# HongjianFang/DSurfTomo

Hardware: AMD Instinct MI355X
Metric: source-period FMM solves/sec on NxN grid; travel-time max-abs-err vs ref (higher is better)
Workload: dtype f32

## Files before the change

### dsurftomo_amd/csrc/bundle_kernel.hip

```cpp
#include "kernels.h"
#include "receiver_core.h"
#include "wave_ops.h"

namespace dsa {

namespace {

__device__ __forceinline__ unsigned bf2u(float f) { return __float_as_uint(f); }
__device__ __forceinline__ float bu2f(unsigned u) { return __uint_as_float(u); }

enum { BC_READY = 0, BC_READY_ODD, BC_TMIN, BC_THETA, BC_FREEZE, BC_HASH, BC_OVERFLOW, BC_CUR, BC_STALE, BC_STALEMIN, BC_SLOWN, BC_FARALL, BC_COUNT };
constexpr int kFarStrikes = 8;
constexpr int kBundleCycleRounds = 8;
constexpr float kStaleWindows = 16.0f;
constexpr int kStaleRounds = 6;

typedef __attribute__((address_space(1))) unsigned long long BGU64;
typedef __attribute__((address_space(1))) char BGChar;
typedef __attribute__((address_space(1))) float BGF32;
typedef __attribute__((address_space(1))) const float BGCF32;
typedef float __attribute__((ext_vector_type(4))) BV4;
typedef __attribute__((address_space(1))) BV4 BGV4;
typedef float __attribute__((ext_vector_type(2))) BV2;
template <int MPL> struct BMem;
// ... 18 lines not shown

template <int CH>
__device__ __forceinline__ unsigned node_or(unsigned v)
{
    if (CH >= 2) v |= (unsigned)__builtin_amdgcn_update_dpp(0, (int)v, 0xb1, 0xf, 0xf, false);
    if (CH >= 4) v |= (unsigned)__builtin_amdgcn_update_dpp(0, (int)v, 0x4e, 0xf, 0xf, false);
    if (CH >= 8) v |= (unsigned)__builtin_amdgcn_update_dpp(0, (int)v, 0x141, 0xf, 0xf, false);
    return v;
}

}

#ifdef DSA_BUNDLE_WAVES
#define DSA_BUNDLE_OCC(G, NT, MPL) __attribute__((amdgpu_waves_per_eu(DSA_BUNDLE_WAVES, DSA_BUNDLE_WAVES)))
#else
#define DSA_BUNDLE_OCC(G, NT, MPL) __attribute__((amdgpu_waves_per_eu((((NT) == 256 && ((MPL) == 2 || (G) == 16)) || (NT) == 768) ? 3 : 1, (((NT) == 256 && ((MPL) == 2 || (G) == 16)) || (NT) == 768) ? 3 : 2)))
#endif
template <int G, int NT, int MPL = 4, bool TIE = false>
__global__ __launch_bounds__(NT) DSA_BUNDLE_OCC(G, NT, MPL) void k_fim_bundle(const FimBundle* __restrict__ bundles, const FimProblem* __restrict__ problems,
                                                    const FimEnds* __restrict__ ends)
{
    constexpr int NW = NT / 64;
    constexpr int CH = G / MPL;
    typedef typename BMem<MPL>::V BV;
    typedef typename BMem<MPL>::GV BGV;
    constexpr int NPW = 64 / CH;
    constexpr unsigned GB = G * 4u * DSA_BSTRIDE;
    extern __shared__ unsigned dyn_lds[];
    __shared__ int sc[BC_COUNT];
    constexpr int kWaveBuf = 256, kTileBuf = NT > 256 ? 128 : 256, kClrWords = 4;
    __shared__ int wbuf[NW * kWaveBuf];
// ... 904 lines not shown
            if (TIE && pm->tie) { pm->tie[4] = freezes; pm->tie[7] = cand_g ? __hip_atomic_load(cand_g, __ATOMIC_RELAXED, __HIP_MEMORY_SCOPE_AGENT) : -1; }
            if (failed && pm->info[2] != -2) pm->info[2] = -1;
            if (sc[BC_OVERFLOW]) pm->info[2] = -2;
        }
        if (E->rays) {
            const GridDesc g = E->g;
            for (int r = tid; r < E->nrays; r += NT) {
                const RayDesc rd = E->rays[r];
                if (!(rd.flags & kRayTime)) continue;
                float t;
                if (!receiver_time(g, E->scx, E->scz, rd, (const float*)Bslot + m, E->veln, E->dpl, &t, G * DSA_BSTRIDE)) atomicExch(E->err, E->ray0 + r + 1);
                E->out[rd.data] = t;
            }
        }
    }
    {
        __shared__ float* s_dst[kBundleMax];
        __syncthreads();
        if (tid < kBundleMax) s_dst[tid] = tid < nmem ? problems[s_member[tid]].Tc : nullptr;
        __syncthreads();
        bool any_dst = false;
        for (int m = 0; m < nmem; ++m) any_dst = any_dst || s_dst[m] != nullptr;
        if (any_dst)
            for (int i = tid; i < ntile * kTileRecs; i += NT) {
#pragma unroll
                for (int c4 = 0; c4 < G / 4; ++c4) {
                    const BV4 v = *(BGV4*)(Bb + (unsigned)i * GB + (unsigned)c4 * 16u);
                    BGF32* d;
                    if ((d = (BGF32*)s_dst[4 * c4 + 0])) d[i] = fabsf(v.x);
                    if ((d = (BGF32*)s_dst[4 * c4 + 1])) d[i] = fabsf(v.y);
                    if ((d = (BGF32*)s_dst[4 * c4 + 2])) d[i] = fabsf(v.z);
                    if ((d = (BGF32*)s_dst[4 * c4 + 3])) d[i] = fabsf(v.w);
// ... 4 lines not shown
        __threadfence();
        __syncthreads();
        if (tid == 0) __hip_atomic_store(&bd->slot_busy[my_slot], 0, __ATOMIC_RELEASE, __HIP_MEMORY_SCOPE_AGENT);
    }
}

size_t bundle_lds_bytes(int tile_words) { return (size_t)tile_words * 4; }

void launch_fim_bundles(const FimBundle* d_bundles, int nbundles, int G, int threads, const FimProblem* d_problems, const FimEnds* d_ends, int tile_words, hipStream_t stream, int members_per_lane, bool tie)
{
    if (nbundles <= 0) return;
    const size_t lds = bundle_lds_bytes(tile_words);
#define DSA_LAUNCH_BUNDLE_T(GG, TT, MM, TIE_) hipLaunchKernelGGL((k_fim_bundle<GG, TT, MM, TIE_>), dim3(nbundles), dim3(TT), lds, stream, d_bundles, d_problems, d_ends)
#define DSA_LAUNCH_BUNDLE_G(TT, MM, TIE_) { if (G == 16) DSA_LAUNCH_BUNDLE_T(16, TT, MM, TIE_); else if (G == 8) DSA_LAUNCH_BUNDLE_T(8, TT, MM, TIE_); else DSA_LAUNCH_BUNDLE_T(4, TT, MM, TIE_); }
#define DSA_LAUNCH_BUNDLE(TT, MM) { if (tie) DSA_LAUNCH_BUNDLE_G(TT, MM, true) else DSA_LAUNCH_BUNDLE_G(TT, MM, false) }
    if (members_per_lane == 2 && threads == 256) DSA_LAUNCH_BUNDLE(256, 2)
    else if (threads == 512) DSA_LAUNCH_BUNDLE(512, 4)
    else if (threads == 768) DSA_LAUNCH_BUNDLE(768, 4)
    else DSA_LAUNCH_BUNDLE(256, 4)
#undef DSA_LAUNCH_BUNDLE_T
#undef DSA_LAUNCH_BUNDLE_G
#undef DSA_LAUNCH_BUNDLE
}

__global__ void k_interleave_maps(const float* __restrict__ slow_all, size_t field_stride, int np, float* __restrict__ slowI)
{
    const size_t i = (size_t)blockIdx.x * blockDim.x + threadIdx.x;
    if (i >= field_stride * (size_t)np) return;
    const size_t id = i / (size_t)np;
    const int m = (int)(i - id * (size_t)np);
    slowI[i] = slow_all[(size_t)m * field_stride + id];
}

template <int G>
__global__ void k_bundle_refined_slowness(const FimBundle* __restrict__ bundles, const FimProblem* __restrict__ problems, int nrec, float* __restrict__ slowI)
{
    const FimBundle* const bd = bundles + blockIdx.y;
    const int i = blockIdx.x * blockDim.x + threadIdx.x;
    if (i >= nrec * G) return;
    const int id = i / G, m = i - id * G;
    const int mm = m < bd->nmem ? m : 0;
    slowI[((size_t)blockIdx.y * nrec + id) * G + m] = problems[bd->member[mm]].slow[id];
}
template <int G>
__global__ void k_bundle_export_records(const FimBundle* __restrict__ bundles, const FimProblem* __restrict__ problems, int nrec)
{
    const FimBundle* const bd = bundles + blockIdx.y;
    const int i = blockIdx.x * blockDim.x + threadIdx.x;
    if (i >= nrec * G) return;
    const int id = i / G, m = i - id * G;
    if (m >= bd->nmem) return;
    const FimProblem* const pm = problems + bd->member[m];
    if (pm->ended && *pm->ended) return;
    const float v = bd->B[(size_t)bd->slot * bd->b_stride + (size_t)id * G * DSA_BSTRIDE + m];
    Rec r{ v, v };
    if (__builtin_signbit(v)) {
        bool pinned = false;
        const float tau = exc_find(bd->exc + (size_t)bd->slot * bd->exc_stride, bd->exc_log2cap, id * G + m, &pinned);
        r.T = pinned ? v : -v; r.tau = tau;
    }
    pm->F[id] = r;
}

void launch_bundle_refined_slowness(const FimBundle* d_bundles, int nbundles, int G, const FimProblem* d_problems, int nrec, float* d_slowI, hipStream_t stream)
{
    if (nbundles <= 0) return;
    const dim3 grid((unsigned)((nrec * G + 255) / 256), (unsigned)nbundles), block(256);
    if (G == 16) hipLaunchKernelGGL(k_bundle_refined_slowness<16>, grid, block, 0, stream, d_bundles, d_problems, nrec, d_slowI);
    else if (G == 8) hipLaunchKernelGGL(k_bundle_refined_slowness<8>, grid, block, 0, stream, d_bundles, d_problems, nrec, d_slowI);
    else hipLaunchKernelGGL(k_bundle_refined_slowness<4>, grid, block, 0, stream, d_bundles, d_problems, nrec, d_slowI);
}

void launch_bundle_export_records(const FimBundle* d_bundles, int nbundles, int G, const FimProblem* d_problems, int nrec, hipStream_t stream)
{
    if (nbundles <= 0) return;
    const dim3 grid((unsigned)((nrec * G + 255) / 256), (unsigned)nbundles), block(256);
    if (G == 16) hipLaunchKernelGGL(k_bundle_export_records<16>, grid, block, 0, stream, d_bundles, d_problems, nrec);
    else if (G == 8) hipLaunchKernelGGL(k_bundle_export_records<8>, grid, block, 0, stream, d_bundles, d_problems, nrec);
    else hipLaunchKernelGGL(k_bundle_export_records<4>, grid, block, 0, stream, d_bundles, d_problems, nrec);
}

void launch_interleave_maps(const float* d_slow_all, size_t field_stride, int np, float* d_slowI, hipStream_t stream)
{
    const size_t n = field_stride * (size_t)np;
    if (n == 0) return;
    hipLaunchKernelGGL(k_interleave_maps, dim3((unsigned)((n + 255) / 256)), dim3(256), 0, stream, d_slow_all, field_stride, np, d_slowI);
}

}
```

### dsurftomo_amd/csrc/engine.h

```cpp
#pragma once

#include <hip/hip_runtime.h>

#include <string>
#include <vector>

#include "bundle_plan.h"
#include "host_geometry.h"
#include "kernels.h"

namespace dsa {

template <class T>
struct DevBuf {
    T* p = nullptr;
    size_t cap = 0;
    void release() { if (p) (void)hipFree(p); p = nullptr; cap = 0; }
};

template <class T>
struct OwnedBuf : DevBuf<T> {
    OwnedBuf() = default;
    OwnedBuf(const OwnedBuf&) = delete;
    OwnedBuf& operator=(const OwnedBuf&) = delete;
// ... 73 lines not shown
    float bundle_window_opt = 0.0f;
    int bundle_G_now = 0;
    int bundle_threads_opt = 0;
    int bundle_max_rounds = 0;
    int bundle_mpl = 0;
    bool bundle_wide = false;
    int bundle_mpl_now = 4, bundle_mpl_b = 2;
    int bundle_threads_b = 256;
    int bundle_tail_opt = 1;
    int bundle_far_all = 0;
    int bundles_a = 0, bundles_b = 0, bundle_Gb = 0;
    hipStream_t stream2 = nullptr;
    hipEvent_t ev_b0 = nullptr, ev_b1 = nullptr;
    hipError_t make_stream2();
    int bundle_refined_opt = 1;
    bool refined_bundles_failed = false;
    bool refined_bundles_now = false;
    std::vector<FimBundle> h_bundles_r;
    OwnedBuf<FimBundle> bundles_r_d;
    OwnedBuf<FimEnds> ends_r;
    OwnedBuf<float> Br_pool, slowIr;
    OwnedBuf<unsigned long long> exc_br;
    OwnedBuf<int> lists_br, cand_br;
    size_t slowIr_off_b = 0;
    int bundle_pool_opt = 0;
    OwnedBuf<float> slowI, B_pool;
    bool slowI_ready = false;
    bool bundles_failed = false;
    OwnedBuf<unsigned long long> exc_b;
    OwnedBuf<int> lists_b, bpool_gen, member_flag, cand_b;
// ... 261 lines not shown
```

### dsurftomo_amd/csrc/engine.hip

```cpp
#include <hip/hip_runtime.h>

#include <algorithm>
#include <chrono>
#include <cmath>
#include <cstdarg>
#include <cstdio>
#include <cstring>
#include <string>
#include <map>
#include <vector>

#include "../../include/dsurftomo_amd.h"
#include "engine.h"
#include "spmv_state.h"
#include "column_system.h"
#include "column_radial.h"
#include "column_lateral.h"
#include "column_radial_lateral.h"
#include "column_sample.h"

namespace dsa {

static std::string g_create_error;

// ... 1311 lines not shown
           b(rst) + b(cst) + b(cinit) + b(heap) + b(flags) + b(T_c) + b(exc_c) + b(W_c) + b(seed_c) + b(nseed_c) + b(launch_rank) + b(prob_r) + b(prob_c) +
           b(info) + b(clocks) + b(tieinfo) + b(xinfo) + b(x_units) + b(B_pool) + b(exc_b) + b(lists_b) + b(bpool_gen) + b(bundles_d) + b(member_flag);
}

float Engine::bundle_window() const
{
    if (bundle_window_opt > 0.0f) return bundle_window_opt;
    if (bundle_wide && bundle_G_now > 0) return bundle_G_now < 16 ? 1.75f : 1.0f;
    return 0.6f;
}

float Engine::bundle_window_tail() const
{
    if (bundle_window_opt > 0.0f) return bundle_window_opt;
    return bundle_threads_b == 768 && bundle_threads() == 256 ? 1.0f : bundle_window();
}

int Engine::bundle_threads() const
{
    if (bundle_threads_opt == 256 || bundle_threads_opt == 512 || bundle_threads_opt == 768) return bundle_threads_opt;
    if (std::max(g.nnx, g.nnz) > 1500) return 768;
    return bundle_wide ? 768 : 256;
}

BundleOptions Engine::bundle_options() const
{
    return { bundle_opt, bundle_mpl, bundle_tail_opt, bundle_order_opt, bundle_threads(), bundle_threads_opt == 0 };
}

BatchPtrs Engine::batch() const
// ... 135 lines not shown
        if (plan_bundles(first, n, bundle_off_chunk ? 0 : bundle_G, &nsolo, &nbundles) != 0) return status;
        const bool refined_b = nbundles > 0 && refined_bundles_now && !bundle_off_chunk;
        const double bundle_mb = nbundles ? (double)(B_pool.cap * 4 + exc_b.cap * 8 + lists_b.cap * 4 + slowI.cap * 4 + cand_b.cap * 4 + Br_pool.cap * 4 + exc_br.cap * 8 + lists_br.cap * 4 + cand_br.cap * 4 + slowIr.cap * 4) / 1.0e6 : 0.0;
        launch_make_problems(g, b, n, slow.p, nrec_c, risti_c.p, window_r, window_c, prob_r.p, prob_c.p, info.p, clocks.p, launch_rank.p,
                             detect ? tieinfo.p : nullptr, tie_threshold, ends_c.p, fused_times ? rays.p : nullptr, veln.p, nfield, dpl, out.p, err.p,
                             nbundles ? member_flag.p : nullptr, bundle_window() * cell_c, bundle_max_rounds, stream, bundle_window_tail() * cell_c,
                             refined_b ? ends_r.p : nullptr);
        FimLaunch sr = shape_r, sc = shape_c;
        sr.tie = sc.tie = detect ? 1 : 0;
        launch_refine(g, b, n, velv.p, (size_t)g.nx * g.ny, rbasis.p, stream);
        if (exact_ties != 2) launch_refined_startup(g, b, n, stream);
        HIP_TRY(this, hipEventRecord(events[2], stream));
        if (exact_ties != 2 && refined_b) {
            launch_fim(prob_r.p, nsolo, sr, stream);
            const int cnt[2] = { bundles_a, nbundles - bundles_a }, GG[2] = { bundle_G, bundle_Gb }, mpl[2] = { bundle_mpl_now, bundles_b > 0 && bundle_threads_b == 256 ? bundle_mpl_b : bundle_mpl_of(bundle_options(), bundle_Gb ? bundle_Gb : bundle_G, nbundles) };
            for (int q = 0; q < 2; ++q) {
                if (cnt[q] <= 0) continue;
                const FimBundle* const bq = bundles_r_d.p + (q ? bundles_a : 0);
                launch_bundle_refined_slowness(bq, cnt[q], GG[q], prob_r.p, kRefRecs, slowIr.p + (q ? slowIr_off_b : 0), stream);
                launch_fim_bundles(bq, cnt[q], GG[q], 256, prob_r.p, ends_r.p, sr.tile_words, stream, GG[q] == 16 ? 4 : mpl[q], detect);
                launch_bundle_export_records(bq, cnt[q], GG[q], prob_r.p, kRefRecs, stream);
            }
        } else if (exact_ties != 2) launch_fim(prob_r.p, n, sr, stream);
        HIP_TRY(this, hipEventRecord(events[3], stream));
        if (exact_ties != 2) {
            const bool replay = detect && handoff_replay;
            if (replay) HIP_TRY(this, hipMemsetAsync(replay_list.p, 0, sizeof(int32_t), stream));
            launch_handoff(g, b, n, stream, detect ? tieinfo.p : nullptr, tie_threshold, replay ? replay_list.p : nullptr, kHandoffReplayCap, replay_scratch.p, xinfo.p);
            launch_coarse_march(g, b, n, slow.p, nrec_c, risti_c.p, stream, detect ? tieinfo.p : nullptr);
        }
        HIP_TRY(this, hipEventRecord(events[4], stream));
        if (exact_ties != 2) {
            launch_fim(prob_c.p, nsolo, sc, stream, ends_c.p);
            if (nbundles && bundles_b > 0) {
                if (!stream2) HIP_TRY(this, make_stream2());
                HIP_TRY(this, hipEventRecord(ev_b0, stream));
                launch_fim_bundles(bundles_d.p, bundles_a, bundle_G, bundle_threads(), prob_c.p, ends_c.p, sc.tile_words, stream, bundle_mpl_now, detect);
                HIP_TRY(this, hipStreamWaitEvent(stream2, ev_b0, 0));
                launch_fim_bundles(bundles_d.p + bundles_a, bundles_b, bundle_Gb, bundle_threads_b, prob_c.p, ends_c.p, sc.tile_words, stream2, bundle_mpl_b, detect);
                HIP_TRY(this, hipEventRecord(ev_b1, stream2));
                HIP_TRY(this, hipStreamWaitEvent(stream, ev_b1, 0));
            } else if (nbundles) launch_fim_bundles(bundles_d.p, nbundles, bundle_G, bundle_threads(), prob_c.p, ends_c.p, sc.tile_words, stream, bundle_mpl_now, detect);
        }
        HIP_TRY(this, hipEventRecord(events[5], stream));
        if (exact_ties) {
            std::vector<int> xl;
            if (exact_ties == 2) { xl.resize((size_t)n); for (int u = 0; u < n; ++u) xl[(size_t)u] = u; }
            else {
                std::vector<int32_t> h_tie((size_t)n * kTieWords), h_inf((size_t)n * 16);
                HIP_TRY(this, hipMemcpyAsync(h_tie.data(), tieinfo.p, (size_t)n * kTieWords * 4, hipMemcpyDeviceToHost, stream));
                HIP_TRY(this, hipMemcpyAsync(h_inf.data(), info.p, (size_t)n * 64, hipMemcpyDeviceToHost, stream));
                int32_t h_replayed = 0;
                if (handoff_replay) HIP_TRY(this, hipMemcpyAsync(&h_replayed, replay_list.p, 4, hipMemcpyDeviceToHost, stream));
                HIP_TRY(this, hipStreamSynchronize(stream));
                stats[DSA_STAT_HANDOFFS_REPLAYED] += (double)std::min<int32_t>(h_replayed, kHandoffReplayCap);
                bool will_redo = false;
                for (int u = 0; u < n && !will_redo; ++u) {
                    const int32_t* fi = &h_inf[(size_t)u * 16];
                    const bool member = nbundles > 0 && h_member_flag[(size_t)u] != 0;
                    will_redo = fi[10] == -2 || (refined_b && member && fi[2] < 0) || (member && fi[10] == -1);
                }
                if (!will_redo) {
                    const std::vector<char> fl = tie_verdicts(first, n, h_tie.data(), h_inf.data(), nbundles > 0);
                    for (int u = 0; u < n; ++u) if (fl[(size_t)u]) { h_unit_flags[(size_t)(first + u)] |= 1; xl.push_back(u); }
                }
                stats[DSA_STAT_TIE_UNITS] += (double)xl.size();
            }
            if (!xl.empty()) {
                const auto w0 = std::chrono::steady_clock::now();
                const bool times_only = !rows && !keep_fields;
                bool compact = exact_ties == 1 ? n <= pool_slots : (!exact_fused || n <= pool_slots);
                if (times_only && exact_tiles_opt == 1) compact = false;
                marched_in_tiles = false;
                if (run_exact(first, n, xl, exact_fused || exact_ties == 1, compact, times_only) != 0) return status;
                stats[DSA_STAT_MS_EXACT] += std::chrono::duration<double, std::milli>(std::chrono::steady_clock::now() - w0).count();
            }
        }
        const int r0 = h_src[first].first_ray;
        const int r1 = h_src[first + n - 1].first_ray + h_src[first + n - 1].nrec;
        if (!fused_times && !exact_fused && r1 > r0) launch_srtimes_chunk(r0, r1 - r0, first);
        HIP_TRY(this, hipEventRecord(events[6], stream));
        HIP_TRY(this, hipGetLastError());
        h_info.resize((size_t)n * 16);
        h_flags.resize((size_t)n * 4);
        std::vector<int32_t> h_tie0;
        if (exact_ties == 0 && detect) { h_tie0.resize((size_t)n * kTieWords); HIP_TRY(this, hipMemcpyAsync(h_tie0.data(), tieinfo.p, (size_t)n * kTieWords * 4, hipMemcpyDeviceToHost, stream)); }
        HIP_TRY(this, hipMemcpyAsync(h_info.data(), info.p, (size_t)n * 16 * 4, hipMemcpyDeviceToHost, stream));
        HIP_TRY(this, hipMemcpyAsync(h_flags.data(), flags.p, (size_t)n * 4 * 4, hipMemcpyDeviceToHost, stream));
        if (dsurf && r1 > r0) {
            const int d0 = h_rays[r0].data, d1 = h_rays[r1 - 1].data + 1;
            HIP_TRY(this, hipMemcpyAsync(dsurf + d0, out.p + d0, (size_t)(d1 - d0) * 4, hipMemcpyDeviceToHost, stream));
        }
        std::vector<unsigned long long> h_clk((size_t)n * kClockSlots);
        HIP_TRY(this, hipMemcpyAsync(h_clk.data(), clocks.p, (size_t)n * kClockSlots * 8, hipMemcpyDeviceToHost, stream));
        HIP_TRY(this, hipStreamSynchronize(stream));
        for (int u = 0; u < n; ++u) {
            for (int q = 0; q < 6; ++q) phase_ticks[q] += (double)h_clk[(size_t)u * kClockSlots + q];
            phase_ticks[7] += (double)h_clk[(size_t)u * kClockSlots + 7];
            phase_ticks[6] = std::max(phase_ticks[6], (double)h_clk[(size_t)u * kClockSlots + 6]);
            for (int q = 8; q < kClockSlots; ++q) phase_ticks[q] += (double)h_clk[(size_t)u * kClockSlots + q];
        }
        float ms = 0;
        float a = 0, c2 = 0, d = 0;
        HIP_TRY(this, hipEventElapsedTime(&ms, events[2], events[3])); stats[DSA_STAT_MS_FIM_REFINED] += ms;
        HIP_TRY(this, hipEventElapsedTime(&ms, events[4], events[5])); stats[DSA_STAT_MS_FIM_COARSE] += ms;
        HIP_TRY(this, hipEventElapsedTime(&a, events[1], events[2]));
        HIP_TRY(this, hipEventElapsedTime(&c2, events[3], events[4]));
        HIP_TRY(this, hipEventElapsedTime(&d, events[5], events[6]));
        stats[DSA_STAT_MS_STAGES] += a + c2 + d;
        stats[DSA_STAT_LAUNCHES_FIM_COARSE] += 1;
        for (int u = 0; u < n; ++u) {
            const int32_t* fi = &h_info[(size_t)u * 16];
            if (fi[10] != -2) continue;
            const size_t grown_bytes = (size_t)pool_slots * (((size_t)8 << (exc_log2cap + 2)) - ((size_t)8 << exc_log2cap));
            size_t free_b = 0, total_b = 0;
            HIP_TRY(this, hipMemGetInfo(&free_b, &total_b));
            if (exc_log2cap + 2 > 26 || grown_bytes + ((size_t)pool_slots << exc_log2cap) * 8 > free_b || ensure(exc_c, (size_t)pool_slots << (exc_log2cap + 2))) {
                fail(DSA_ERR_INTERNAL, "unit %d: the exception table of the compact field overflowed (%d entries) and cannot grow", first + u, 1 << exc_log2cap);
                return DSA_ERR_INTERNAL;
            }
            exc_log2cap += 2;
            exc_log2cap_grown = exc_log2cap;
            per_slot_bytes += grown_bytes / (size_t)pool_slots;
            stats[DSA_STAT_RESCANS] += 1;
// ... 662 lines not shown
    if (n == "fim_lds_pad" && value >= 0 && value <= 64 * 1024) { en->planned = false; en->fim_lds_pad = (int)value; return 0; }
    if (n == "fim_sorted" && (value == 0 || value == 1)) { en->planned = false; en->fim_sorted = (int)value; return 0; }
    if (n == "ray_path_cap" && value >= 0 && value <= (1 << 24)) { en->ray_path_cap = (int)value; return 0; }
    if (n == "disp_group_shift" && value >= -1 && value <= 3) { en->disp_group_shift = (int)value; return 0; }
    if (n == "disp_layers_lds" && (value == -1 || value == 0 || value == 1)) { en->disp_layers_lds = (int)value; return 0; }
    if (n == "exc_log2cap" && (value == 0 || (value >= 6 && value <= 24))) { en->planned = false; en->exc_log2cap_opt = (int)value; return 0; }
    if (n == "rows_on_device" && (value == 0 || value == 1)) { en->rows_on_device = value != 0; return 0; }
    if (n == "lsmr_device_vectors" && (value == 0 || value == 1)) { en->lsmr_device_vectors = (int)value; return 0; }
    if (n == "field_pool" && value >= -1) { en->planned = false; en->field_pool_opt = (int)value; return 0; }
    if (n == "ray_lanes" && (value == 0 || value == 1 || value == 4)) { en->ray_lanes_opt = (int)value; return 0; }
    if (n == "bundle_window_cells" && value >= 0) { en->bundle_window_opt = (float)value; return 0; }
    if (n == "bundle_threads" && (value == 0 || value == 256 || value == 512 || value == 768)) { en->bundle_threads_opt = (int)value; return 0; }
    if (n == "bundle_max_rounds" && value >= 0) { en->bundle_max_rounds = (int)value; return 0; }
    if (n == "bundle_tail" && (value == 0 || value == 1)) { en->bundle_tail_opt = (int)value; return 0; }
    if (n == "bundle_refined" && (value == 0 || value == 1 || value == 2)) { en->bundle_refined_opt = (int)value; return 0; }
    if (n == "bundle_far_all" && (value == 0 || value == 1)) { en->bundle_far_all = (int)value; return 0; }
    if (n == "bundle_pool" && value >= 0) { en->bundle_pool_opt = (int)value; return 0; }
    if (n == "bundle_members_per_lane" && (value == 0 || value == 4 || value == 2)) { en->bundle_mpl = (int)value; return 0; }
    if (n == "bundle" && (value == 0 || value == 1 || value == 4 || value == 8 || value == 16)) { en->planned = false; en->bundle_opt = (int)value; return 0; }
    if (n == "exact_ties" && (value == 0 || value == 1 || value == 2)) { en->exact_ties = (int)value; return 0; }
    if (n == "tie_threshold" && value >= 0) { en->tie_threshold = (float)value; return 0; }
    if (n == "tie_detect" && (value == 0 || value == 1)) { en->tie_detect = (int)value; return 0; }
    if (n == "tie_sum_threshold" && value >= 0) { en->tie_sum_threshold = (float)value; return 0; }
    if (n == "tie_count_threshold" && value >= 0) { en->tie_count_threshold = (int)value; return 0; }
    if (n == "tie_frozen_bundles" && (value == 0 || value == 1)) { en->tie_frozen_bundles = (int)value; return 0; }
    if (n == "tie_map_strict" && (value == 0 || value == 1)) { en->tie_map_strict = (int)value; return 0; }
    if (n == "tie_scale_guard" && (value == 0 || value == 1)) { en->tie_scale_guard = (int)value; return 0; }
    if (n == "handoff_replay" && (value == 0 || value == 1)) { en->handoff_replay = (int)value; return 0; }
    if (n == "tie_tolerance" && value > 0) { en->tie_tolerance = (float)value; return 0; }
    if (n == "bundle_order" && (value == 0 || value == 1 || value == 2 || value == 3)) { en->bundle_order_opt = (int)value; return 0; }
// ... 487 lines not shown
```

### dsurftomo_amd/csrc/kernels.h

```cpp
#pragma once

#include <hip/hip_runtime.h>
#include <stdint.h>

#include "source_stage.h"

namespace dsa {

struct RayDesc { int src; float rx, rz; float sin_rx; int data; int flags; };
constexpr int kRayTime = 1, kRayPath = 2;

constexpr int kClockSlots = 32;
constexpr int kTieWords = 16;
constexpr float kTieSumUnit = 0x1p-30f;
constexpr int kTieSeenLog2 = 14, kTieSeenSlots = 1 << kTieSeenLog2;

struct FimProblem {
    Rec* F;
    float* Tc;
    unsigned long long* exc;
    int exc_log2cap;
    const float* slow;
    const float* risti;
    const int* seed;
// ... 119 lines not shown
constexpr int kReplayHeap = 4096;
constexpr size_t handoff_replay_bytes() { return (size_t)kReplayHeap * 8; }
void launch_refined_replay(const GridDesc& g, const BatchPtrs& b, const int32_t* d_list, int cap, void* d_heap, int gcap, int32_t* d_xinfo, hipStream_t stream);
void launch_coarse_march(const GridDesc& g, const BatchPtrs& b, int nsrc, const float* d_slow_all,
                         size_t field_stride, const float* d_risti_c, hipStream_t stream, int32_t* d_tie = nullptr );
void launch_make_problems(const GridDesc& g, const BatchPtrs& b, int nsrc, const float* d_slow_all,
                          size_t field_stride, const float* d_risti_c, float window_r, float window_c,
                          FimProblem* d_prob_r, FimProblem* d_prob_c, int32_t* d_info, unsigned long long* d_clocks,
                          const int* d_launch_rank, int32_t* d_tie, float tie_threshold, FimEnds* d_ends_c, const RayDesc* d_rays ,
                          const float* d_veln_all, size_t veln_stride, float dpl, float* d_out, int32_t* d_err,
                          const int* d_member_flag , float window_b ,
                          int max_rounds_b , hipStream_t stream,
                          float window_t = 0.0f ,
                          FimEnds* d_ends_r = nullptr );
void launch_bundle_refined_slowness(const FimBundle* d_bundles, int nbundles, int G, const FimProblem* d_problems, int nrec, float* d_slowI, hipStream_t stream);
void launch_bundle_export_records(const FimBundle* d_bundles, int nbundles, int G, const FimProblem* d_problems, int nrec, hipStream_t stream);

size_t exact_lds_bytes(int lcap);
size_t exact_heap_blocked_entries(int lcap, int gcap);
size_t exact_start_bytes();
struct XTiles { void* tt; void* tp; void* ring; void* freestk; void* pins; int tcap; };
size_t exact_tile_table_entries(int ntile);
size_t exact_tile_unit_bytes(int ntile, int tcap);
struct XReceivers { const RayDesc* rays; const float* veln_all; size_t veln_stride; float dpl; float* out; int32_t* err; };
void launch_exact(const GridDesc& g, const BatchPtrs& b, const int* d_units, int n, const float* d_slow_all, size_t field_stride,
                  const float* d_risti_c, void* d_pool, size_t pool_stride, void* d_heap_pool, int gcap, int lcap, void* d_starts, int* d_nstart,
                  int32_t* d_xinfo, unsigned long long* d_clocks ,
                  const XReceivers* receivers , bool compact_copy , hipStream_t stream,
                  const XTiles* tiles = nullptr ,
                  int gstride = 0 , int lb = 0 );

// ... 126 lines not shown
```

### dsurftomo_amd/csrc/stage_kernels.hip

```cpp
#include "kernels.h"
#include "receiver_core.h"
#include "exact_march.h"
#include "radial_system.h"

namespace dsa {

namespace {

__device__ __forceinline__ SourceScratch scratch_of(const BatchPtrs& b, int s)
{
    SourceScratch w;
    const size_t rr = (size_t)kRefMax * kRefMax;
    w.slow_r = b.slow_r + (size_t)s * kRefRecs;
    w.F_r = b.F_r + (size_t)s * kRefRecs;
    w.S_r = b.S_r + s * rr;
    w.risti_r = b.risti_r + (size_t)s * kRefMax;
    w.vcorner = b.vcorner + (size_t)s * 4;
    w.rst = b.rst + (size_t)s * kRWin * kRWin;
    w.cst = b.cst + (size_t)s * kCWinMax * kCWinMax;
    w.cinit = b.cinit + (size_t)s * kCWinMax * kCWinMax;
    w.heap = b.heap + (size_t)s * kHeapCap;
    w.flags = b.flags + (size_t)s * 4;
    return w;
}
// ... 216 lines not shown
    for (int q = tid; q < bxn * bzn; q += nt) {
        const int cx = sd.vnl + q / bzn, cz = sd.vnt + q % bzn;
        int16_t* me = &w.cst[(cx - 1 - sd.cwx0) * sd.cwnz + (cz - 1 - sd.cwz0)];
        if (*me != 0) continue;
        const int nx[4] = { cx - 1, cx + 1, cx, cx }, nz[4] = { cz, cz, cz - 1, cz + 1 };
        bool band = false;
        for (int d = 0; d < 4; ++d) {
            if (nx[d] < 1 || nx[d] > g.nnx || nz[d] < 1 || nz[d] > g.nnz) continue;
            const bool inwin = nz[d] > sd.cwz0 && nz[d] <= sd.cwz0 + sd.cwnz && nx[d] > sd.cwx0 && nx[d] <= sd.cwx0 + sd.cwnx;
            if (!inwin || w.cst[(nx[d] - 1 - sd.cwx0) * sd.cwnz + (nz[d] - 1 - sd.cwz0)] == -1) band = true;
        }
        if (band) *me = 1;
    }
}

__global__ __launch_bounds__(256) void k_handoff(GridDesc g, BatchPtrs b)
{
    __shared__ unsigned long long s_best;
    __shared__ int s_first;
    handoff_unit(g, b, blockIdx.x, s_best, s_first);
}

__global__ __launch_bounds__(256) void k_handoff_probe(GridDesc g, BatchPtrs b, int32_t* tie, float tie_threshold, int32_t* replay, int replay_cap)
{
    constexpr int kTiedMax = 8;
    __shared__ int s_tied[kTiedMax], s_ntied;
    const int s = blockIdx.x, tid = threadIdx.x;
    const SourceDesc sd = b.src[s];
    SourceScratch w = scratch_of(b, s);
    const int ended = w.flags[0], ez = w.flags[2], ex = w.flags[3];
    if (tid == 0) s_ntied = 0;
    __syncthreads();
    if (ended || ex <= 0) return;
    const int n = sd.rnx * sd.rnz, eid = (ex - 1) * sd.rnz + (ez - 1);
    const Rec er = w.F_r[rec_index(sd.nbz_r, ez - 1, ex - 1)];
    const uint64_t rstar = accept_rank(er.T, er.tau);
    {
        const int dq = 256 / sd.rnz, dr = 256 % sd.rnz;
        int ix0 = tid / sd.rnz, iz0 = tid % sd.rnz;
        for (int id = tid; id < n; id += 256) {
            const Rec r = w.F_r[rec_index(sd.nbz_r, iz0, ix0)];
            if (id != eid && !t_pinned(r.T) && t_value(r.T) < kInf && accept_rank(r.T, r.tau) == rstar) { const int k = atomicAdd(&s_ntied, 1); if (k < kTiedMax) s_tied[k] = id; }
// ... 47 lines not shown
        if (!(zx >= 1 && zx <= sd.rnx && zz >= 1 && zz <= sd.rnz && (zx - 1) % kSgdl == 0 && (zz - 1) % kSgdl == 0)) continue;
        float t1;
        const int st1 = handoff_node<true>(g, sd, w, 0, rstar, ez, ex, zz, zx, &t1, yid);
        const int zid = (zx - 1) * sd.rnz + (zz - 1);
        const int st0 = w.S_r[zid];
        const float t0 = Tfin[zid];
        if (st1 != st0) atomicAdd(tr + 6, 1);
        else if (st0 >= 0 && t1 != t0) {
            const float ti = fabsf(t1 - t0);
            atomicAdd((unsigned*)tr + 2, 1u); atomicAdd((unsigned*)tr + 3, (unsigned)(fminf(ti, 1.0f) * (1.0f / kTieSumUnit)));
            if (ti > tie_threshold) { atomicAdd((unsigned*)tr, 1u); atomicMax((unsigned*)tr + 1, __float_as_uint(ti)); }
        }
    }
}

static_assert(sizeof(XRec) == sizeof(Rec) && sizeof(XEntry) == 8, "the march's records lie where the fixed point's do");

__global__ __launch_bounds__(64) void k_handoff_replay(GridDesc g, BatchPtrs b, const int32_t* replay, int replay_cap, const int32_t* xinfo, int32_t* tie)
{
    __shared__ unsigned long long s_best;
    __shared__ int s_first;
    const int j = blockIdx.x, lane = threadIdx.x;
    const int cnt = replay[0] < replay_cap ? replay[0] : replay_cap;
    if (j >= cnt) return;
    const int s = replay[1 + j];
    const SourceDesc sd = b.src[s];
    SourceScratch w = scratch_of(b, s);
    if (xinfo[4 * s + 2]) { if (lane == 0) atomicAdd(tie + (size_t)s * kTieWords + 6, 1); return; }
    for (int ix = 0; ix < sd.rnx; ++ix)
        for (int iz = lane; iz < sd.rnz; iz += 64) {
            const int id = rec_index(sd.nbz_r, iz, ix);
            const XRec r = reinterpret_cast<const XRec*>(w.F_r)[id];
            w.F_r[id] = r.st == 0 ? Rec{ -r.T, r.T } : r.st > 0 ? Rec{ r.T, r.T } : Rec{ kInf, kInf };
        }
    if (lane == 0) w.flags[0] = 1;
    __threadfence_block();
    __syncthreads();
    handoff_unit(g, b, s, s_best, s_first);
}

void launch_handoff(const GridDesc& g, const BatchPtrs& b, int nsrc, hipStream_t stream, int32_t* d_tie, float tie_threshold, int32_t* d_replay, int replay_cap, void* d_replay_scratch,
                    int32_t* d_xinfo)
{
    if (nsrc <= 0) return;
    hipLaunchKernelGGL(k_handoff, dim3(nsrc), dim3(256), 0, stream, g, b);
    const bool replay = d_tie && d_replay && replay_cap > 0 && d_replay_scratch && d_xinfo;
    if (d_tie) hipLaunchKernelGGL(k_handoff_probe, dim3(nsrc), dim3(256), 0, stream, g, b, d_tie, tie_threshold, replay ? d_replay : nullptr, replay_cap);
    if (replay) {
        launch_refined_replay(g, b, d_replay, replay_cap, d_replay_scratch, kReplayHeap, d_xinfo, stream);
        hipLaunchKernelGGL(k_handoff_replay, dim3(replay_cap), dim3(64), 0, stream, g, b, (const int32_t*)d_replay, replay_cap, (const int32_t*)d_xinfo, d_tie);
    }
}

__global__ __launch_bounds__(64) void k_coarse_march(GridDesc g, BatchPtrs b, int nsrc, const float* __restrict__ slow_all,
                                                     size_t field_stride, const float* __restrict__ risti_c, int32_t* tie)
{
    const int s = blockIdx.x, lane = threadIdx.x;
    if (s >= nsrc) return;
    const SourceDesc sd = b.src[s];
    SourceScratch w = scratch_of(b, s);
    Rec* W = b.W_c + (size_t)s * kCWinMax * kCWinMax;
    const float* slow_c = slow_all + (size_t)sd.period * field_stride;
// ... 177 lines not shown
```

### dsurftomo_amd/engine.py

```python
import ctypes as C
import os

import numpy as np

_HERE = os.path.dirname(os.path.abspath(__file__))
LIB_PATH = os.environ.get("DSA_LIB_PATH") or os.path.join(_HERE, "libdsurftomo_amd.so")

STAT_NAMES = ("ms_total", "ms_fim_coarse", "ms_fim_refined", "ms_stages", "launches_fim_coarse", "units",
              "rounds_max", "evals_total", "chunk", "rescans", "freezes", "rays", "ray_steps", "rays_clamped",
              "ms_rays", "ms_rows", "nar", "ms_dispersion", "curves", "changes_total", "tie_units", "exact_units", "exact_pops", "ms_exact", "field_slots", "footprint_mb", "bundle_size", "bundles", "bundled_units", "bundle_slots", "bundle_threads", "tie_units_left", "tie_influence_max", "exact_pool", "exact_tiles", "tie_units_strict", "tie_prone_maps", "tie_units_tied", "tie_units_by_scale", "handoffs_replayed", "ray_launches")

_f32, _i32, _vp = C.c_float, C.c_int, C.c_void_p
_lib = None


class EngineError(RuntimeError):
    def __init__(self, code, text):
        super().__init__("dsurftomo_amd error %d: %s" % (code, text))
        self.code = code


def load_library():
    global _lib
    if _lib is not None:
        return _lib
# ... 771 lines not shown
```

### include/dsurftomo_amd.h

```cpp
#ifndef DSURFTOMO_AMD_H
#define DSURFTOMO_AMD_H

#include <stddef.h>
#include <stdint.h>

#ifdef __cplusplus
extern "C" {
#endif

typedef struct dsa_engine dsa_engine;

enum dsa_status {
    DSA_OK = 0,
    DSA_ERR_DEVICE = -1,
    DSA_ERR_ARGUMENT = -2,
    DSA_ERR_OUTSIDE = -3,
    DSA_ERR_INTERNAL = -4,
    DSA_ERR_STATE = -5,
    DSA_ERR_CAPACITY = -6
};

int dsa_create(dsa_engine** out, int device_index);
void dsa_destroy(dsa_engine* e);
const char* dsa_error_string(const dsa_engine* e);
// ... 177 lines not shown
       DSA_STAT_CHUNK, DSA_STAT_RESCANS, DSA_STAT_FREEZES, DSA_STAT_RAYS, DSA_STAT_RAY_STEPS,
       DSA_STAT_RAYS_CLAMPED, DSA_STAT_MS_RAYS, DSA_STAT_MS_ROWS, DSA_STAT_NAR, DSA_STAT_MS_DISPERSION,
       DSA_STAT_CURVES, DSA_STAT_CHANGES_TOTAL, DSA_STAT_TIE_UNITS, DSA_STAT_EXACT_UNITS, DSA_STAT_EXACT_POPS,
       DSA_STAT_MS_EXACT, DSA_STAT_FIELD_SLOTS, DSA_STAT_FOOTPRINT_MB, DSA_STAT_BUNDLE_SIZE, DSA_STAT_BUNDLES,
       DSA_STAT_BUNDLED_UNITS, DSA_STAT_BUNDLE_SLOTS, DSA_STAT_BUNDLE_THREADS,
       DSA_STAT_TIE_UNITS_LEFT,
       DSA_STAT_TIE_INFLUENCE_MAX,
       DSA_STAT_EXACT_POOL,
       DSA_STAT_EXACT_TILES,
       DSA_STAT_TIE_UNITS_STRICT,
       DSA_STAT_TIE_PRONE_MAPS,
       DSA_STAT_TIE_UNITS_TIED,
       DSA_STAT_TIE_UNITS_BY_SCALE,
       DSA_STAT_HANDOFFS_REPLAYED,
       DSA_STAT_RAY_LAUNCHES,
       DSA_STAT_COUNT };
int dsa_get_stats(const dsa_engine* e, double* out );

int dsa_calsurfg(const int* nx, const int* ny, const int* nz, const int* nparpi, const float* vels,
                 int* iw, float* rw, int* col, float* dsurf,
                 const float* goxdf, const float* gozdf, const float* dvxdf, const float* dvzdf,
                 const int* kmaxRc, const int* kmaxRg, const int* kmaxLc, const int* kmaxLg,
                 const double* tRc, const double* tRg, const double* tLc, const double* tLg,
                 const int* wavetype, const int* igrt, const int* periods, const float* depz,
                 const float* minthk, const float* scxf, const float* sczf, const float* rcxf,
                 const float* rczf, const int* nrc1, const int* nsrcsurf1, const int* kmax,
                 const int* nsrcsurf, const int* nrcf, int* nar);

int dsa_synthetic(const int* nx, const int* ny, const int* nz, const int* nparpi, const float* vels,
                  float* obst,
// ... 66 lines not shown
```

Before: 45210.

## Fuse refined record export and handoff probe, add 128-thread refined bundles

Moves the refined record export into the tail of the bundle kernel, removing the separate export kernel. It also merges the handoff and probe kernels into one templated launch, and runs the two refined bundle groups concurrently on a second stream, or as a single launch when their shapes match. It adds a 128-thread bundle variant chosen for mid-sized bundle counts, and batches the host tail copies so the exact-ties path needs only one synchronize. Each piece cuts launch count or host sync overhead, at the cost of more work inside the bundle kernel and extra stream-ordering complexity.

Result: faster. 45910, median of 6 (+1.5%).

```diff
diff --git a/dsurftomo_amd/csrc/bundle_kernel.hip b/dsurftomo_amd/csrc/bundle_kernel.hip
--- a/dsurftomo_amd/csrc/bundle_kernel.hip
+++ b/dsurftomo_amd/csrc/bundle_kernel.hip
@@ -56,7 +56,8 @@
 #ifdef DSA_BUNDLE_WAVES
 #define DSA_BUNDLE_OCC(G, NT, MPL) __attribute__((amdgpu_waves_per_eu(DSA_BUNDLE_WAVES, DSA_BUNDLE_WAVES)))
 #else
-#define DSA_BUNDLE_OCC(G, NT, MPL) __attribute__((amdgpu_waves_per_eu((((NT) == 256 && ((MPL) == 2 || (G) == 16)) || (NT) == 768) ? 3 : 1, (((NT) == 256 && ((MPL) == 2 || (G) == 16)) || (NT) == 768) ? 3 : 2)))
+#define DSA_BUNDLE_OCC3(G, NT, MPL) ((((NT) == 256 || (NT) == 128) && ((MPL) == 2 || (G) == 16)) || (NT) == 768)
+#define DSA_BUNDLE_OCC(G, NT, MPL) __attribute__((amdgpu_waves_per_eu(DSA_BUNDLE_OCC3(G, NT, MPL) ? 3 : 1, DSA_BUNDLE_OCC3(G, NT, MPL) ? 3 : 2)))
 #endif
 template <int G, int NT, int MPL = 4, bool TIE = false>
 __global__ __launch_bounds__(NT) DSA_BUNDLE_OCC(G, NT, MPL) void k_fim_bundle(const FimBundle* __restrict__ bundles, const FimProblem* __restrict__ problems,
@@ -991,8 +992,38 @@
             }
         }
     }
+    __shared__ float* s_dst[kBundleMax];
+    if (ends[s_member[0]].Fpin) {
+        __syncthreads();
+        if (tid < kBundleMax) {
+            const FimProblem* const pm = problems + s_member[tid];
+            s_dst[tid] = tid < nmem && !(pm->ended && *pm->ended) ? (float*)pm->F : nullptr;
+        }
+        __syncthreads();
+        typedef __attribute__((address_space(1))) BV2 BGRec;
+        static_assert(sizeof(Rec) == sizeof(BV2), "a record is two floats");
+        for (int i = tid; i < ntile * kTileRecs; i += NT) {
+#pragma unroll
+            for (int c4 = 0; c4 < G / 4; ++c4) {
+                const BV4 v4 = *(BGV4*)(Bb + (unsigned)i * GB + (unsigned)c4 * 16u);
+                const float vv[4] = { v4.x, v4.y, v4.z, v4.w };
+#pragma unroll
+                for (int j = 0; j < 4; ++j) {
+                    BGRec* const d = (BGRec*)s_dst[4 * c4 + j];
+                    if (!d) continue;
+                    const float v = vv[j];
+                    BV2 r = { v, v };
+                    if (__builtin_signbit(v)) {
+                        bool pinned = false;
+                        const float tau = exc_lookup(i * G + 4 * c4 + j, &pinned);
+                        r.x = pinned ? v : -v; r.y = tau;
+                    }
+                    d[i] = r;
+                }
+            }
+        }
+    }
     {
-        __shared__ float* s_dst[kBundleMax];
         __syncthreads();
         if (tid < kBundleMax) s_dst[tid] = tid < nmem ? problems[s_member[tid]].Tc : nullptr;
         __syncthreads();
@@ -1027,7 +1058,8 @@
 #define DSA_LAUNCH_BUNDLE_T(GG, TT, MM, TIE_) hipLaunchKernelGGL((k_fim_bundle<GG, TT, MM, TIE_>), dim3(nbundles), dim3(TT), lds, stream, d_bundles, d_problems, d_ends)
 #define DSA_LAUNCH_BUNDLE_G(TT, MM, TIE_) { if (G == 16) DSA_LAUNCH_BUNDLE_T(16, TT, MM, TIE_); else if (G == 8) DSA_LAUNCH_BUNDLE_T(8, TT, MM, TIE_); else DSA_LAUNCH_BUNDLE_T(4, TT, MM, TIE_); }
 #define DSA_LAUNCH_BUNDLE(TT, MM) { if (tie) DSA_LAUNCH_BUNDLE_G(TT, MM, true) else DSA_LAUNCH_BUNDLE_G(TT, MM, false) }
-    if (members_per_lane == 2 && threads == 256) DSA_LAUNCH_BUNDLE(256, 2)
+    if (threads == 128) DSA_LAUNCH_BUNDLE(128, 4)
+    else if (members_per_lane == 2 && threads == 256) DSA_LAUNCH_BUNDLE(256, 2)
     else if (threads == 512) DSA_LAUNCH_BUNDLE(512, 4)
     else if (threads == 768) DSA_LAUNCH_BUNDLE(768, 4)
     else DSA_LAUNCH_BUNDLE(256, 4)
@@ -1055,26 +1087,6 @@
     const int mm = m < bd->nmem ? m : 0;
     slowI[((size_t)blockIdx.y * nrec + id) * G + m] = problems[bd->member[mm]].slow[id];
 }
-template <int G>
-__global__ void k_bundle_export_records(const FimBundle* __restrict__ bundles, const FimProblem* __restrict__ problems, int nrec)
-{
-    const FimBundle* const bd = bundles + blockIdx.y;
-    const int i = blockIdx.x * blockDim.x + threadIdx.x;
-    if (i >= nrec * G) return;
-    const int id = i / G, m = i - id * G;
-    if (m >= bd->nmem) return;
-    const FimProblem* const pm = problems + bd->member[m];
-    if (pm->ended && *pm->ended) return;
-    const float v = bd->B[(size_t)bd->slot * bd->b_stride + (size_t)id * G * DSA_BSTRIDE + m];
-    Rec r{ v, v };
-    if (__builtin_signbit(v)) {
-        bool pinned = false;
-        const float tau = exc_find(bd->exc + (size_t)bd->slot * bd->exc_stride, bd->exc_log2cap, id * G + m, &pinned);
-        r.T = pinned ? v : -v; r.tau = tau;
-    }
-    pm->F[id] = r;
-}
-
 void launch_bundle_refined_slowness(const FimBundle* d_bundles, int nbundles, int G, const FimProblem* d_problems, int nrec, float* d_slowI, hipStream_t stream)
 {
     if (nbundles <= 0) return;
@@ -1084,15 +1096,6 @@
     else hipLaunchKernelGGL(k_bundle_refined_slowness<4>, grid, block, 0, stream, d_bundles, d_problems, nrec, d_slowI);
 }
 
-void launch_bundle_export_records(const FimBundle* d_bundles, int nbundles, int G, const FimProblem* d_problems, int nrec, hipStream_t stream)
-{
-    if (nbundles <= 0) return;
-    const dim3 grid((unsigned)((nrec * G + 255) / 256), (unsigned)nbundles), block(256);
-    if (G == 16) hipLaunchKernelGGL(k_bundle_export_records<16>, grid, block, 0, stream, d_bundles, d_problems, nrec);
-    else if (G == 8) hipLaunchKernelGGL(k_bundle_export_records<8>, grid, block, 0, stream, d_bundles, d_problems, nrec);
-    else hipLaunchKernelGGL(k_bundle_export_records<4>, grid, block, 0, stream, d_bundles, d_problems, nrec);
-}
-
 void launch_interleave_maps(const float* d_slow_all, size_t field_stride, int np, float* d_slowI, hipStream_t stream)
 {
     const size_t n = field_stride * (size_t)np;
diff --git a/dsurftomo_amd/csrc/engine.h b/dsurftomo_amd/csrc/engine.h
--- a/dsurftomo_amd/csrc/engine.h
+++ b/dsurftomo_amd/csrc/engine.h
@@ -111,6 +111,8 @@
     hipEvent_t ev_b0 = nullptr, ev_b1 = nullptr;
     hipError_t make_stream2();
     int bundle_refined_opt = 1;
+    int bundle_refined_threads_opt = 0;
+    int refined_bundle_threads(int nbundles, int G) const;
     bool refined_bundles_failed = false;
     bool refined_bundles_now = false;
     std::vector<FimBundle> h_bundles_r;
diff --git a/dsurftomo_amd/csrc/engine.hip b/dsurftomo_amd/csrc/engine.hip
--- a/dsurftomo_amd/csrc/engine.hip
+++ b/dsurftomo_amd/csrc/engine.hip
@@ -1349,6 +1349,12 @@
 {
     if (bundle_window_opt > 0.0f) return bundle_window_opt;
     return bundle_threads_b == 768 && bundle_threads() == 256 ? 1.0f : bundle_window();
+}
+
+int Engine::refined_bundle_threads(int nbundles, int G) const
+{
+    if (bundle_refined_threads_opt) return bundle_refined_threads_opt;
+    return nbundles > 768 && nbundles <= (G == 16 ? 1280 : 1024) ? 128 : 256;
 }
 
 int Engine::bundle_threads() const
@@ -1514,13 +1520,23 @@
         if (exact_ties != 2 && refined_b) {
             launch_fim(prob_r.p, nsolo, sr, stream);
             const int cnt[2] = { bundles_a, nbundles - bundles_a }, GG[2] = { bundle_G, bundle_Gb }, mpl[2] = { bundle_mpl_now, bundles_b > 0 && bundle_threads_b == 256 ? bundle_mpl_b : bundle_mpl_of(bundle_options(), bundle_Gb ? bundle_Gb : bundle_G, nbundles) };
-            for (int q = 0; q < 2; ++q) {
-                if (cnt[q] <= 0) continue;
-                const FimBundle* const bq = bundles_r_d.p + (q ? bundles_a : 0);
-                launch_bundle_refined_slowness(bq, cnt[q], GG[q], prob_r.p, kRefRecs, slowIr.p + (q ? slowIr_off_b : 0), stream);
-                launch_fim_bundles(bq, cnt[q], GG[q], 256, prob_r.p, ends_r.p, sr.tile_words, stream, GG[q] == 16 ? 4 : mpl[q], detect);
-                launch_bundle_export_records(bq, cnt[q], GG[q], prob_r.p, kRefRecs, stream);
-            }
+            const int thr = refined_bundle_threads(nbundles, std::max(GG[0], GG[1]));
+            const auto refined_group = [&](int k0, int count, int G_, int mpl_, hipStream_t st) {
+                const FimBundle* const bq = bundles_r_d.p + k0;
+                launch_bundle_refined_slowness(bq, count, G_, prob_r.p, kRefRecs, slowIr.p + (k0 ? slowIr_off_b : 0), st);
+                launch_fim_bundles(bq, count, G_, thr, prob_r.p, ends_r.p, sr.tile_words, st, mpl_, detect);
+            };
+            const int mr[2] = { GG[0] == 16 || thr == 128 ? 4 : mpl[0], GG[1] == 16 || thr == 128 ? 4 : mpl[1] };
+            if (cnt[0] > 0 && cnt[1] > 0 && GG[0] == GG[1] && mr[0] == mr[1]) refined_group(0, nbundles, GG[0], mr[0], stream);
+            else if (cnt[0] > 0 && cnt[1] > 0) {
+                if (!stream2) HIP_TRY(this, make_stream2());
+                HIP_TRY(this, hipEventRecord(ev_b0, stream));
+                refined_group(0, cnt[0], GG[0], mr[0], stream);
+                HIP_TRY(this, hipStreamWaitEvent(stream2, ev_b0, 0));
+                refined_group(bundles_a, cnt[1], GG[1], mr[1], stream2);
+                HIP_TRY(this, hipEventRecord(ev_b1, stream2));
+                HIP_TRY(this, hipStreamWaitEvent(stream, ev_b1, 0));
+            } else for (int q = 0; q < 2; ++q) if (cnt[q] > 0) refined_group(q ? bundles_a : 0, cnt[q], GG[q], mr[q], stream);
         } else if (exact_ties != 2) launch_fim(prob_r.p, n, sr, stream);
         HIP_TRY(this, hipEventRecord(events[3], stream));
         if (exact_ties != 2) {
@@ -1543,16 +1559,37 @@
             } else if (nbundles) launch_fim_bundles(bundles_d.p, nbundles, bundle_G, bundle_threads(), prob_c.p, ends_c.p, sc.tile_words, stream, bundle_mpl_now, detect);
         }
         HIP_TRY(this, hipEventRecord(events[5], stream));
+        const int r0 = h_src[first].first_ray;
+        const int r1 = h_src[first + n - 1].first_ray + h_src[first + n - 1].nrec;
+        h_info.resize((size_t)n * 16);
+        h_flags.resize((size_t)n * 4);
+        std::vector<unsigned long long> h_clk((size_t)n * kClockSlots);
+        const auto copy_tail = [&](bool info_first) -> hipError_t {
+            hipError_t rc = hipSuccess;
+            if (info_first) rc = hipMemcpyAsync(h_info.data(), info.p, (size_t)n * 16 * 4, hipMemcpyDeviceToHost, stream);
+            if (rc == hipSuccess) rc = hipEventRecord(events[6], stream);
+            if (rc == hipSuccess && !info_first) rc = hipMemcpyAsync(h_info.data(), info.p, (size_t)n * 16 * 4, hipMemcpyDeviceToHost, stream);
+            if (rc == hipSuccess) rc = hipMemcpyAsync(h_flags.data(), flags.p, (size_t)n * 4 * 4, hipMemcpyDeviceToHost, stream);
+            if (rc == hipSuccess && dsurf && r1 > r0) {
+                const int d0 = h_rays[r0].data, d1 = h_rays[r1 - 1].data + 1;
+                rc = hipMemcpyAsync(dsurf + d0, out.p + d0, (size_t)(d1 - d0) * 4, hipMemcpyDeviceToHost, stream);
+            }
+            if (rc == hipSuccess) rc = hipMemcpyAsync(h_clk.data(), clocks.p, (size_t)n * kClockSlots * 8, hipMemcpyDeviceToHost, stream);
+            return rc;
+        };
+        bool tail_copied = false;
         if (exact_ties) {
             std::vector<int> xl;
             if (exact_ties == 2) { xl.resize((size_t)n); for (int u = 0; u < n; ++u) xl[(size_t)u] = u; }
             else {
-                std::vector<int32_t> h_tie((size_t)n * kTieWords), h_inf((size_t)n * 16);
+                std::vector<int32_t> h_tie((size_t)n * kTieWords);
+                const std::vector<int32_t>& h_inf = h_info;
                 HIP_TRY(this, hipMemcpyAsync(h_tie.data(), tieinfo.p, (size_t)n * kTieWords * 4, hipMemcpyDeviceToHost, stream));
-                HIP_TRY(this, hipMemcpyAsync(h_inf.data(), info.p, (size_t)n * 64, hipMemcpyDeviceToHost, stream));
                 int32_t h_replayed = 0;
                 if (handoff_replay) HIP_TRY(this, hipMemcpyAsync(&h_replayed, replay_list.p, 4, hipMemcpyDeviceToHost, stream));
+                HIP_TRY(this, copy_tail(true));
                 HIP_TRY(this, hipStreamSynchronize(stream));
+                tail_copied = true;
                 stats[DSA_STAT_HANDOFFS_REPLAYED] += (double)std::min<int32_t>(h_replayed, kHandoffReplayCap);
                 bool will_redo = false;
                 for (int u = 0; u < n && !will_redo; ++u) {
@@ -1572,28 +1609,19 @@
                 bool compact = exact_ties == 1 ? n <= pool_slots : (!exact_fused || n <= pool_slots);
                 if (times_only && exact_tiles_opt == 1) compact = false;
                 marched_in_tiles = false;
+                tail_copied = false;
                 if (run_exact(first, n, xl, exact_fused || exact_ties == 1, compact, times_only) != 0) return status;
                 stats[DSA_STAT_MS_EXACT] += std::chrono::duration<double, std::milli>(std::chrono::steady_clock::now() - w0).count();
             }
         }
-        const int r0 = h_src[first].first_ray;
-        const int r1 = h_src[first + n - 1].first_ray + h_src[first + n - 1].nrec;
         if (!fused_times && !exact_fused && r1 > r0) launch_srtimes_chunk(r0, r1 - r0, first);
-        HIP_TRY(this, hipEventRecord(events[6], stream));
         HIP_TRY(this, hipGetLastError());
-        h_info.resize((size_t)n * 16);
-        h_flags.resize((size_t)n * 4);
         std::vector<int32_t> h_tie0;
-        if (exact_ties == 0 && detect) { h_tie0.resize((size_t)n * kTieWords); HIP_TRY(this, hipMemcpyAsync(h_tie0.data(), tieinfo.p, (size_t)n * kTieWords * 4, hipMemcpyDeviceToHost, stream)); }
-        HIP_TRY(this, hipMemcpyAsync(h_info.data(), info.p, (size_t)n * 16 * 4, hipMemcpyDeviceToHost, stream));
-        HIP_TRY(this, hipMemcpyAsync(h_flags.data(), flags.p, (size_t)n * 4 * 4, hipMemcpyDeviceToHost, stream));
-        if (dsurf && r1 > r0) {
-            const int d0 = h_rays[r0].data, d1 = h_rays[r1 - 1].data + 1;
-            HIP_TRY(this, hipMemcpyAsync(dsurf + d0, out.p + d0, (size_t)(d1 - d0) * 4, hipMemcpyDeviceToHost, stream));
-        }
-        std::vector<unsigned long long> h_clk((size_t)n * kClockSlots);
-        HIP_TRY(this, hipMemcpyAsync(h_clk.data(), clocks.p, (size_t)n * kClockSlots * 8, hipMemcpyDeviceToHost, stream));
-        HIP_TRY(this, hipStreamSynchronize(stream));
+        if (!tail_copied) {
+            HIP_TRY(this, copy_tail(false));
+            if (exact_ties == 0 && detect) { h_tie0.resize((size_t)n * kTieWords); HIP_TRY(this, hipMemcpyAsync(h_tie0.data(), tieinfo.p, (size_t)n * kTieWords * 4, hipMemcpyDeviceToHost, stream)); }
+            HIP_TRY(this, hipStreamSynchronize(stream));
+        }
         for (int u = 0; u < n; ++u) {
             for (int q = 0; q < 6; ++q) phase_ticks[q] += (double)h_clk[(size_t)u * kClockSlots + q];
             phase_ticks[7] += (double)h_clk[(size_t)u * kClockSlots + 7];
@@ -1608,6 +1636,7 @@
         HIP_TRY(this, hipEventElapsedTime(&c2, events[3], events[4]));
         HIP_TRY(this, hipEventElapsedTime(&d, events[5], events[6]));
         stats[DSA_STAT_MS_STAGES] += a + c2 + d;
+        stats[DSA_STAT_MS_STAGES_SOURCE] += a; stats[DSA_STAT_MS_STAGES_HANDOFF] += c2; stats[DSA_STAT_MS_STAGES_TAIL] += d;
         stats[DSA_STAT_LAUNCHES_FIM_COARSE] += 1;
         for (int u = 0; u < n; ++u) {
             const int32_t* fi = &h_info[(size_t)u * 16];
@@ -2300,6 +2329,7 @@
     if (n == "bundle_max_rounds" && value >= 0) { en->bundle_max_rounds = (int)value; return 0; }
     if (n == "bundle_tail" && (value == 0 || value == 1)) { en->bundle_tail_opt = (int)value; return 0; }
     if (n == "bundle_refined" && (value == 0 || value == 1 || value == 2)) { en->bundle_refined_opt = (int)value; return 0; }
+    if (n == "bundle_refined_threads" && (value == 0 || value == 128 || value == 256)) { en->bundle_refined_threads_opt = (int)value; return 0; }
     if (n == "bundle_far_all" && (value == 0 || value == 1)) { en->bundle_far_all = (int)value; return 0; }
     if (n == "bundle_pool" && value >= 0) { en->bundle_pool_opt = (int)value; return 0; }
     if (n == "bundle_members_per_lane" && (value == 0 || value == 4 || value == 2)) { en->bundle_mpl = (int)value; return 0; }
diff --git a/dsurftomo_amd/csrc/kernels.h b/dsurftomo_amd/csrc/kernels.h
--- a/dsurftomo_amd/csrc/kernels.h
+++ b/dsurftomo_amd/csrc/kernels.h
@@ -157,7 +157,6 @@
                           float window_t = 0.0f ,
                           FimEnds* d_ends_r = nullptr );
 void launch_bundle_refined_slowness(const FimBundle* d_bundles, int nbundles, int G, const FimProblem* d_problems, int nrec, float* d_slowI, hipStream_t stream);
-void launch_bundle_export_records(const FimBundle* d_bundles, int nbundles, int G, const FimProblem* d_problems, int nrec, hipStream_t stream);
 
 size_t exact_lds_bytes(int lcap);
 size_t exact_heap_blocked_entries(int lcap, int gcap);
diff --git a/dsurftomo_amd/csrc/stage_kernels.hip b/dsurftomo_amd/csrc/stage_kernels.hip
--- a/dsurftomo_amd/csrc/stage_kernels.hip
+++ b/dsurftomo_amd/csrc/stage_kernels.hip
@@ -254,18 +254,12 @@
     }
 }
 
-__global__ __launch_bounds__(256) void k_handoff(GridDesc g, BatchPtrs b)
-{
-    __shared__ unsigned long long s_best;
-    __shared__ int s_first;
-    handoff_unit(g, b, blockIdx.x, s_best, s_first);
-}
-
-__global__ __launch_bounds__(256) void k_handoff_probe(GridDesc g, BatchPtrs b, int32_t* tie, float tie_threshold, int32_t* replay, int replay_cap)
+
+__device__ __forceinline__ void handoff_probe_unit(const GridDesc& g, const BatchPtrs& b, int s, int32_t* tie, float tie_threshold, int32_t* replay, int replay_cap)
 {
     constexpr int kTiedMax = 8;
     __shared__ int s_tied[kTiedMax], s_ntied;
-    const int s = blockIdx.x, tid = threadIdx.x;
+    const int tid = threadIdx.x;
     const SourceDesc sd = b.src[s];
     SourceScratch w = scratch_of(b, s);
     const int ended = w.flags[0], ez = w.flags[2], ex = w.flags[3];
@@ -343,6 +337,19 @@
     }
 }
 
+template <bool PROBE>
+__global__ __launch_bounds__(256) void k_handoff(GridDesc g, BatchPtrs b, int32_t* tie, float tie_threshold, int32_t* replay, int replay_cap)
+{
+    __shared__ unsigned long long s_best;
+    __shared__ int s_first;
+    handoff_unit(g, b, blockIdx.x, s_best, s_first);
+    if (PROBE) {
+        __threadfence_block();
+        __syncthreads();
+        handoff_probe_unit(g, b, blockIdx.x, tie, tie_threshold, replay, replay_cap);
+    }
+}
+
 static_assert(sizeof(XRec) == sizeof(Rec) && sizeof(XEntry) == 8, "the march's records lie where the fixed point's do");
 
 __global__ __launch_bounds__(64) void k_handoff_replay(GridDesc g, BatchPtrs b, const int32_t* replay, int replay_cap, const int32_t* xinfo, int32_t* tie)
@@ -372,9 +379,9 @@
                     int32_t* d_xinfo)
 {
     if (nsrc <= 0) return;
-    hipLaunchKernelGGL(k_handoff, dim3(nsrc), dim3(256), 0, stream, g, b);
     const bool replay = d_tie && d_replay && replay_cap > 0 && d_replay_scratch && d_xinfo;
-    if (d_tie) hipLaunchKernelGGL(k_handoff_probe, dim3(nsrc), dim3(256), 0, stream, g, b, d_tie, tie_threshold, replay ? d_replay : nullptr, replay_cap);
+    if (d_tie) hipLaunchKernelGGL(k_handoff<true>, dim3(nsrc), dim3(256), 0, stream, g, b, d_tie, tie_threshold, replay ? d_replay : nullptr, replay_cap);
+    else hipLaunchKernelGGL(k_handoff<false>, dim3(nsrc), dim3(256), 0, stream, g, b, (int32_t*)nullptr, 0.0f, (int32_t*)nullptr, 0);
     if (replay) {
         launch_refined_replay(g, b, d_replay, replay_cap, d_replay_scratch, kReplayHeap, d_xinfo, stream);
         hipLaunchKernelGGL(k_handoff_replay, dim3(replay_cap), dim3(64), 0, stream, g, b, (const int32_t*)d_replay, replay_cap, (const int32_t*)d_xinfo, d_tie);
diff --git a/dsurftomo_amd/engine.py b/dsurftomo_amd/engine.py
--- a/dsurftomo_amd/engine.py
+++ b/dsurftomo_amd/engine.py
@@ -8,7 +8,8 @@
 
 STAT_NAMES = ("ms_total", "ms_fim_coarse", "ms_fim_refined", "ms_stages", "launches_fim_coarse", "units",
               "rounds_max", "evals_total", "chunk", "rescans", "freezes", "rays", "ray_steps", "rays_clamped",
-              "ms_rays", "ms_rows", "nar", "ms_dispersion", "curves", "changes_total", "tie_units", "exact_units", "exact_pops", "ms_exact", "field_slots", "footprint_mb", "bundle_size", "bundles", "bundled_units", "bundle_slots", "bundle_threads", "tie_units_left", "tie_influence_max", "exact_pool", "exact_tiles", "tie_units_strict", "tie_prone_maps", "tie_units_tied", "tie_units_by_scale", "handoffs_replayed", "ray_launches")
+              "ms_rays", "ms_rows", "nar", "ms_dispersion", "curves", "changes_total", "tie_units", "exact_units", "exact_pops", "ms_exact", "field_slots", "footprint_mb", "bundle_size", "bundles", "bundled_units", "bundle_slots", "bundle_threads", "tie_units_left", "tie_influence_max", "exact_pool", "exact_tiles", "tie_units_strict", "tie_prone_maps", "tie_units_tied", "tie_units_by_scale", "handoffs_replayed", "ray_launches",
+              "ms_stages_source", "ms_stages_handoff", "ms_stages_tail")
 
 _f32, _i32, _vp = C.c_float, C.c_int, C.c_void_p
 _lib = None
diff --git a/include/dsurftomo_amd.h b/include/dsurftomo_amd.h
--- a/include/dsurftomo_amd.h
+++ b/include/dsurftomo_amd.h
@@ -215,6 +215,9 @@
        DSA_STAT_TIE_UNITS_BY_SCALE,
        DSA_STAT_HANDOFFS_REPLAYED,
        DSA_STAT_RAY_LAUNCHES,
+       DSA_STAT_MS_STAGES_SOURCE,
+       DSA_STAT_MS_STAGES_HANDOFF,
+       DSA_STAT_MS_STAGES_TAIL,
        DSA_STAT_COUNT };
 int dsa_get_stats(const dsa_engine* e, double* out );
 
```
